# fhausmann/deepgrp

Hardware: AMD Instinct MI355X
Metric: Mbp/sec predicted (whole node) at window=200 stride=50, 5-class (higher is better)
Workload: dtype f16

## Files before the change

### deepgrp_amd/csrc/gru_shared.h

```cpp
#pragma once
#include "dgrp_model.h"

typedef _Float16 half8 __attribute__((ext_vector_type(8)));
typedef float f32x16 __attribute__((ext_vector_type(16)));
typedef float f32x4 __attribute__((ext_vector_type(4)));
typedef _Float16 half4 __attribute__((ext_vector_type(4)));

#define DGRP_WG_WINDOWS 16

struct gru_rec {
    int64_t idx_off, n, out_row, nwin;
    dgrp_placement place;
    int64_t win_first;
    int64_t pad_;
};

struct gru_params {
    const uint8_t *idx;
    int64_t n, s, w0, nw;
    dgrp_placement place;
    const uint4 *pack;
    const float *ffb;
    float *out;
    void *avg;
    int avg_f32;
    int T, C, nfrag, mode;
    int Tp;
    int ospan;
    const struct gru_rec *recs;
    const int64_t *wg_first;
    int64_t nrec;
    int64_t avgw;
    const uint4 *pack_lo;
    int lo_tile_off;
    float zfold;
    const uint4 *pack16;
    const float *xtab;
    int xtab_off;
    const uint4 *stream;
    const uint4 *packw;
    const float *xtabw;
    int avg_up;
};

__device__ __forceinline__ float sigmoid_from_scaled(float a) { return __builtin_amdgcn_rcpf(1.0f + __builtin_amdgcn_exp2f(a)); }
__device__ __forceinline__ float tanh_from_scaled(float a) { return 1.0f - 2.0f * __builtin_amdgcn_rcpf(1.0f + __builtin_amdgcn_exp2f(a)); }
typedef float f32x2 __attribute__((ext_vector_type(2)));
__device__ __forceinline__ f32x2 rcp1p_exp2_pair(float a0, float a1)
{
    f32x2 e = { __builtin_amdgcn_exp2f(a0), __builtin_amdgcn_exp2f(a1) };
    e = e + 1.0f;
    return f32x2{ __builtin_amdgcn_rcpf(e.x), __builtin_amdgcn_rcpf(e.y) };
}
__device__ __forceinline__ float fast_tanh(float x) { return tanh_from_scaled(2.8853900817779268f * x); }

template <int N>
__device__ __forceinline__ float row_ror(float x)
{
    return __builtin_bit_cast(float, __builtin_amdgcn_update_dpp(0, __builtin_bit_cast(int, x), 0x120 | N, 0xf, 0xf, false));
}
template <int N>
__device__ __forceinline__ float row_max_ror(float x)
{
    float r;
    asm("s_nop 1\n\tv_max_f32_dpp %0, %1, %1 row_ror:%2 row_mask:0xf bank_mask:0xf" : "=v"(r) : "v"(x), "n"(N));
    return r;
}
template <int CTRL>
__device__ __forceinline__ float quad_perm(float x)
{
    return __builtin_bit_cast(float, __builtin_amdgcn_update_dpp(0, __builtin_bit_cast(int, x), CTRL, 0xf, 0xf, false));
}
__device__ __forceinline__ float row_allmax(float x)
{
    return row_max_ror<1>(row_max_ror<2>(row_max_ror<4>(row_max_ror<8>(x))));
}
__device__ __forceinline__ float row_allsum(float x)
{
    x += row_ror<8>(x); x += row_ror<4>(x); x += row_ror<2>(x); return x + row_ror<1>(x);
}

typedef __attribute__((address_space(3))) unsigned lds_u32;
typedef __attribute__((address_space(1))) unsigned glb_u32;
__device__ __forceinline__ void lds_atomic_max(unsigned *p, unsigned v)
{
    (void)__hip_atomic_fetch_max((lds_u32 *)p, v, __ATOMIC_RELAXED, __HIP_MEMORY_SCOPE_WORKGROUP);
}
__device__ __forceinline__ void global_atomic_max(unsigned *p, unsigned v)
{
    (void)__hip_atomic_fetch_max((glb_u32 *)p, v, __ATOMIC_RELAXED, __HIP_MEMORY_SCOPE_AGENT);
}

__host__ __device__ static inline int gru_lds_hbuf(int UP, int pad = 8) { return 2 * 32 * (UP + pad) * 2; }
__host__ __device__ static inline int gru_lds_dpart(int NW) { return 2 * NW * 64 * 16; }
__host__ __device__ static inline int gru_lds_seq(int Tp) { return DGRP_WG_WINDOWS * Tp; }
__host__ __device__ static inline int gru_lds_meta() { return DGRP_WG_WINDOWS * 8 + DGRP_WG_WINDOWS * 4; }

struct wg_ctx {
    _Float16 *hbuf;
    float *dpart;
    uint8_t *seqs;
    int64_t *row0s;
    int *rowoff;
    unsigned *obuf;
    int64_t wg_w, lo;
    int nvalid;
};

template <int MODE>
__device__ __forceinline__ int64_t wg_record_at(const gru_params &pin, gru_params &p, int64_t g)
{
    if (MODE == 1 || !pin.recs) return g;
    int64_t lo_r = 0, hi_r = pin.nrec;
    while (hi_r - lo_r > 1) {
        const int64_t mid = (lo_r + hi_r) >> 1;
        if (pin.wg_first[mid] <= g) lo_r = mid; else hi_r = mid;
    }
    const gru_rec rc = pin.recs[lo_r];
    p.idx = pin.idx + rc.idx_off;
    p.n = rc.n;
    if (MODE == 0) p.out = pin.out + rc.out_row * pin.C;
    p.place = rc.place;
    p.w0 = 0;
    p.nw = rc.nwin;
    p.avgw = rc.win_first;
    return g - pin.wg_first[lo_r];
}
template <int MODE>
__device__ __forceinline__ int64_t wg_record(const gru_params &pin, gru_params &p) { return wg_record_at<MODE>(pin, p, blockIdx.x); }

template <int NW, int MODE, int HPAD = 8>
__device__ __forceinline__ wg_ctx wg_setup(const gru_params &p, unsigned char *smem, int64_t bid)
{
    constexpr int UP = 32 * NW, HS = UP + HPAD;
    wg_ctx c;
    c.hbuf = reinterpret_cast<_Float16 *>(smem);
    c.dpart = reinterpret_cast<float *>(smem + gru_lds_hbuf(UP, HPAD));
    c.seqs = smem + gru_lds_hbuf(UP, HPAD) + gru_lds_dpart(NW);
    c.row0s = reinterpret_cast<int64_t *>(c.seqs + gru_lds_seq(p.Tp));
    c.rowoff = reinterpret_cast<int *>(c.row0s + DGRP_WG_WINDOWS);
    c.obuf = reinterpret_cast<unsigned *>(c.rowoff + DGRP_WG_WINDOWS);
    const int tid = threadIdx.x, T = p.T, C = p.C;
    c.wg_w = p.w0 + bid * DGRP_WG_WINDOWS;
    c.nvalid = (int)min((int64_t)DGRP_WG_WINDOWS, p.w0 + p.nw - c.wg_w);
    for (int i = tid; i < DGRP_WG_WINDOWS * T; i += 64 * NW) {
        const int wi = i / T, t = i - wi * T;
        c.seqs[wi * p.Tp + t] = wi < c.nvalid ? p.idx[(c.wg_w + wi) * p.s + t] : (uint8_t)4;
    }
    for (int i = tid; i < 32 * HS; i += 64 * NW) c.hbuf[i] = (_Float16)0.0f;
    c.lo = 0;
    if (MODE == 0) {
        const int64_t a = dgrp_place_row(p.place, c.wg_w, p.s), b = dgrp_place_row(p.place, c.wg_w + c.nvalid - 1, p.s);
        c.lo = a < b ? a : b;
        for (int i = tid; i < p.ospan * C; i += 64 * NW) c.obuf[i] = 0u;
    }
    if (tid < DGRP_WG_WINDOWS) {
        int64_t r0 = -1;
        int off = -1;
        if (tid < c.nvalid) {
            r0 = MODE == 0 ? dgrp_place_row(p.place, c.wg_w + tid, p.s) : (c.wg_w + tid - p.w0 + p.avgw) * (int64_t)T;
            if (MODE == 0 && r0 >= c.lo && r0 - c.lo + T <= p.ospan) off = (int)(r0 - c.lo);
        }
        c.row0s[tid] = r0;
        c.rowoff[tid] = off;
    }
    __syncthreads();
    return c;
}

template <int MODE>
__device__ __forceinline__ void emit_value(const gru_params &p, const wg_ctx &c, int off, int64_t row0, int t, int cls, float val)
{
    if (MODE == 0) {
        if (off >= 0) {
            lds_atomic_max(c.obuf + (off + t) * p.C + cls, __float_as_uint(val));
        } else {
            const int64_t row = row0 + t;
            if (row < p.n) global_atomic_max(reinterpret_cast<unsigned *>(p.out) + row * p.C + cls, __float_as_uint(val));
        }
    } else {
        p.out[(row0 + t) * p.C + cls] = val;
    }
}

template <int NW, int MODE>
__device__ __forceinline__ void finish_register(const gru_params &p, const wg_ctx &c, int t, int reg, float fbias, int off, int64_t row0)
{
    const int lane = threadIdx.x & 63, cls = lane & 15;
    const float *dp = c.dpart + ((size_t)(t & 1) * 4 + reg) * NW * 64 + lane;
    float sum = dp[0];
#pragma unroll
    for (int w = 1; w < NW; ++w) sum += dp[w * 64];
    const int wi = 4 * (lane >> 4) + reg;
    const float lg = cls < p.C ? sum + fbias : -INFINITY;
    float val = lg;
    if (MODE != 2) {
        const float m = row_allmax(lg);
        const float e = __builtin_amdgcn_exp2f(1.4426950408889634f * (lg - m));
        val = e * __builtin_amdgcn_rcpf(row_allsum(e));
    }
    if (cls < p.C && wi < c.nvalid) emit_value<MODE>(p, c, off, row0, t, cls, val);
}

template <int NW>
__device__ __forceinline__ void flush_image(const gru_params &p, const wg_ctx &c)
{
    __syncthreads();
    unsigned *gout = reinterpret_cast<unsigned *>(p.out) + c.lo * p.C;
    const int64_t lim = (p.n - c.lo) * p.C;
    for (int i = threadIdx.x; i < p.ospan * p.C; i += 64 * NW) {
        const unsigned v = c.obuf[i];
        if (v != 0u && i < lim) global_atomic_max(gout + i, v);
    }
}

__device__ __forceinline__ void split_avg_store_lane(const gru_params &p, int64_t wg_w, int tt, int UP, int wave, int lane, half8 a0, half8 a1,
                                                     half8 l0, half8 l1)
{
    const int64_t at = ((wg_w + (lane & 15) - p.w0 + p.avgw) * (int64_t)p.T + tt) * UP + 32 * wave + 8 * (lane >> 4);
    if (p.avg_f32) {
        float *dst = reinterpret_cast<float *>(p.avg) + at;
        typedef unsigned u32x4_ __attribute__((ext_vector_type(4)));
        const _Float16 hf = (_Float16)0.5f;
        const u32x4_ A0 = __builtin_bit_cast(u32x4_, a0), A1 = __builtin_bit_cast(u32x4_, a1);
        const u32x4_ L0 = __builtin_bit_cast(u32x4_, l0 * hf), L1 = __builtin_bit_cast(u32x4_, l1 * hf);
        float v[8];
#pragma unroll
        for (int k = 0; k < 4; ++k) {
            float f0, f1, r0, r1;
            asm("v_fma_mix_f32 %0, %1, 0.5, %2 op_sel_hi:[1,0,1]" : "=v"(f0) : "v"(A0[k]), "v"(L0[k]));
            asm("v_fma_mix_f32 %0, %1, 0.5, %2 op_sel:[1,0,1] op_sel_hi:[1,0,1]" : "=v"(f1) : "v"(A0[k]), "v"(L0[k]));
            asm("v_fma_mix_f32 %0, %1, 0.5, %2 op_sel_hi:[1,0,1]" : "=v"(r0) : "v"(A1[k]), "v"(L1[k]));
            asm("v_fma_mix_f32 %0, %1, 0.5, %2 op_sel:[1,0,1] op_sel_hi:[1,0,1]" : "=v"(r1) : "v"(A1[k]), "v"(L1[k]));
            v[2 * k] = f0 + r0;
            v[2 * k + 1] = f1 + r1;
        }
        *reinterpret_cast<f32x4 *>(dst) = f32x4{ v[0], v[1], v[2], v[3] };
        *reinterpret_cast<f32x4 *>(dst + 4) = f32x4{ v[4], v[5], v[6], v[7] };
        return;
    }
    const _Float16 hf = (_Float16)0.5f;
    const half8 av = (a0 * hf + a1 * hf) + (l0 + l1) * hf;
    *reinterpret_cast<half8 *>(reinterpret_cast<_Float16 *>(p.avg) + at) = av;
}
__device__ __forceinline__ void split_avg_store(const gru_params &p, int64_t wg_w, int tt, int UP, int wave, half8 a0, half8 a1,
                                                half8 l0, half8 l1)
{
    split_avg_store_lane(p, wg_w, tt, UP, wave, threadIdx.x & 63, a0, a1, l0, l1);
}

struct split_gate_tmp { float er, e2, g, A, zt, d, n; };
template <bool ONERCP, int OP>
__device__ __forceinline__ void split_gate_op(split_gate_tmp &t, float ar, float ag, float az, float ax, float &s)
{
#pragma clang fp contract(off)
    if constexpr (OP == 0) t.er = __builtin_amdgcn_exp2f(ar);
    else if constexpr (OP == 1) t.e2 = __builtin_amdgcn_exp2f(az);
    else if constexpr (OP == 2) t.er = t.er + 1.0f;
    else if constexpr (OP == 3) t.er = __builtin_amdgcn_rcpf(t.er);
    else if constexpr (OP == 4) t.g = __builtin_fmaf(t.er, ag, ax);
    else if constexpr (OP == 5) t.A = __builtin_amdgcn_exp2f(t.g);
    else if constexpr (OP == 6) t.A = t.A + 1.0f;
    else if constexpr (ONERCP) {
        if constexpr (OP == 7) t.zt = __builtin_fmaf(0.5f, t.e2, 1.0f);
        else if constexpr (OP == 8) t.d = t.A * t.zt;
        else if constexpr (OP == 9) t.n = __builtin_fmaf(s, t.A, -t.e2);
        else if constexpr (OP == 10) t.d = __builtin_amdgcn_rcpf(t.d);
        else s = t.n * t.d;
    } else {
        if constexpr (OP == 7) t.zt = t.e2 + 1.0f;
        else if constexpr (OP == 8) t.d = __builtin_amdgcn_rcpf(t.A);
        else if constexpr (OP == 9) t.n = __builtin_fmaf(-2.0f, t.d, 1.0f);
        else if constexpr (OP == 10) t.zt = __builtin_amdgcn_rcpf(t.zt);
        else { const float df = s - t.n; s = __builtin_fmaf(t.zt, df, t.n); }
    }
}
#define DGRP_SPLIT_GATE_OPS 12
template <bool ONERCP>
__device__ __forceinline__ float split_gate_chain(float ar, float ag, float az, float ax, float s)
{
    split_gate_tmp t;
    split_gate_op<ONERCP, 0>(t, ar, ag, az, ax, s); split_gate_op<ONERCP, 1>(t, ar, ag, az, ax, s);
    split_gate_op<ONERCP, 2>(t, ar, ag, az, ax, s); split_gate_op<ONERCP, 3>(t, ar, ag, az, ax, s);
    split_gate_op<ONERCP, 4>(t, ar, ag, az, ax, s); split_gate_op<ONERCP, 5>(t, ar, ag, az, ax, s);
    split_gate_op<ONERCP, 6>(t, ar, ag, az, ax, s); split_gate_op<ONERCP, 7>(t, ar, ag, az, ax, s);
    split_gate_op<ONERCP, 8>(t, ar, ag, az, ax, s); split_gate_op<ONERCP, 9>(t, ar, ag, az, ax, s);
    split_gate_op<ONERCP, 10>(t, ar, ag, az, ax, s); split_gate_op<ONERCP, 11>(t, ar, ag, az, ax, s);
    return s;
}
template <bool ONERCP> __device__ __forceinline__ float split_state_h(float s)
{
#pragma clang fp contract(off)
    return ONERCP ? s + 1.0f : s;
}
__device__ __forceinline__ uint2 split_pack4(const float h[4])
{
    uint2 r;
    asm("v_cvt_pk_f16_f32 %0, %1, %2" : "=v"(r.x) : "v"(h[0]), "v"(h[1]));
    asm("v_cvt_pk_f16_f32 %0, %1, %2" : "=v"(r.y) : "v"(h[2]), "v"(h[3]));
    return r;
}
__device__ __forceinline__ void split_residual4(float h[4], uint2 hi)
{
    asm("v_fma_mix_f32 %0, %1, -1.0, %0 op_sel_hi:[1,0,0]" : "+v"(h[0]) : "v"(hi.x));
    asm("v_fma_mix_f32 %0, %1, -1.0, %0 op_sel:[1,0,0] op_sel_hi:[1,0,0]" : "+v"(h[1]) : "v"(hi.x));
    asm("v_fma_mix_f32 %0, %1, -1.0, %0 op_sel_hi:[1,0,0]" : "+v"(h[2]) : "v"(hi.y));
    asm("v_fma_mix_f32 %0, %1, -1.0, %0 op_sel:[1,0,0] op_sel_hi:[1,0,0]" : "+v"(h[3]) : "v"(hi.y));
}
__device__ __forceinline__ void split_hi_lo4(const float h[4], uint2 &hv, uint2 &lv)
{
    float r[4] = { h[0], h[1], h[2], h[3] };
    hv = split_pack4(r);
    split_residual4(r, hv);
    lv = split_pack4(r);
}

__device__ __forceinline__ float wave_half_sum(float h, float half)
{
#pragma clang fp contract(off)
    float t = half * h;
    asm("s_nop 1\n\tv_fmac_f32_dpp %0, %1, %2 row_ror:8 row_mask:0xf bank_mask:0xf" : "+v"(t) : "v"(h), "v"(half));
    return t;
}

__device__ __forceinline__ void split_lstm_cell(float ai, float af, float ac, float ao, float &c, float &h)
{
#pragma clang fp contract(off)
    const float ig = __builtin_amdgcn_rcpf(1.0f + __builtin_amdgcn_exp2f(ai));
    const float fg = __builtin_amdgcn_rcpf(1.0f + __builtin_amdgcn_exp2f(af));
    const float tc = __builtin_fmaf(-2.0f, __builtin_amdgcn_rcpf(1.0f + __builtin_amdgcn_exp2f(ac)), 1.0f);
    const float it = ig * tc;
    c = __builtin_fmaf(fg, c, it);
    const float og = __builtin_amdgcn_rcpf(1.0f + __builtin_amdgcn_exp2f(ao));
    const float e2 = __builtin_amdgcn_exp2f(2.8853900817779268f * c);
    const float th = __builtin_fmaf(-2.0f, __builtin_amdgcn_rcpf(1.0f + e2), 1.0f);
    h = og * th;
}
```

### deepgrp_amd/csrc/gru_split2.hip

```cpp
#include "gru_shared.h"
#include <mutex>
#include <type_traits>

typedef unsigned u32x4 __attribute__((ext_vector_type(4)));

namespace {

constexpr int NW = 4, UP = 128, KS = 4, HPAD = 16, HS = UP + HPAD;
constexpr int XT_PITCH = 4 * 128 * 4 + 32;

struct split2_weights {
    u32x4 hi[3][KS][2], lo[3][KS][2];
    u32x4 Bd_hi, Bd_lo;
};

#define LOAD2(a, pa, b, pb)                                                                                             \
    asm volatile("global_load_dwordx4 %0, %2, off\n\tglobal_load_dwordx4 %1, %3, off\n\ts_waitcnt vmcnt(0)"            \
                 : "=&a"(a), "=&a"(b) : "v"(pa), "v"(pb) : "memory")

#define MFMA_R(acc, Wf, b) asm volatile("v_mfma_f32_16x16x32_f16 %0, %1, %2, %0" : "+v"(acc) : "a"(Wf), "v"(b))
#define MFMA_D(acc, a, Wf) asm volatile("v_mfma_f32_16x16x32_f16 %0, %1, %2, %0" : "+v"(acc) : "v"(a), "a"(Wf))
#define MFMA_DZ(acc, a, Wf) asm volatile("v_mfma_f32_16x16x32_f16 %0, %1, %2, 0" : "=&v"(acc) : "v"(a), "a"(Wf))

struct tile_state {
    gru_params p;
    wg_ctx ctx;
    unsigned hcur, hnxt, lcur, lnxt;
    unsigned myseq;
    float h[16];
    f32x4 ar[4], ag[4], az[4], ax[4];
    f32x4 dpl;
    unsigned tabf, tabr;
    half8 f0h[2], f0l[2];
    int p_off;
    int64_t p_row0;
    bool pr_on;
};

template <int MODE, bool ONERCP>
__global__ void __launch_bounds__(256) __attribute__((amdgpu_waves_per_eu(1, 1))) gru_split2_kernel(const gru_params pin, int half_bytes)
{
    extern __shared__ __attribute__((aligned(16))) unsigned char smem[];
    const int tid = threadIdx.x;
    const int lane = tid & 63;
    const int wave = __builtin_amdgcn_readfirstlane(tid >> 6);
    const int T = pin.T, C = pin.C;

    split2_weights W;
    {
        const uint4 *p16 = pin.pack16 + (size_t)wave * 48 * 64 + lane;
#pragma unroll
        for (int g = 0; g < 3; ++g)
#pragma unroll
            for (int ks = 0; ks < KS; ++ks) {
                LOAD2(W.hi[g][ks][0], p16 + (size_t)(g * 8 + ks * 2) * 64, W.hi[g][ks][1], p16 + (size_t)(g * 8 + ks * 2 + 1) * 64);
                LOAD2(W.lo[g][ks][0], p16 + (size_t)(24 + g * 8 + ks * 2) * 64, W.lo[g][ks][1], p16 + (size_t)(24 + g * 8 + ks * 2 + 1) * 64);
            }
        const uint4 *mypack = pin.pack + (size_t)wave * pin.nfrag * 64 + lane;
        LOAD2(W.Bd_hi, mypack + (size_t)(3 * (2 * KS + 1) + 1) * 64, W.Bd_lo, mypack + (size_t)(3 * (2 * KS + 1) + 2) * 64);
    }
    for (int i = tid; i < 5 * 512; i += 256)
        *reinterpret_cast<float *>(smem + pin.xtab_off + (i / 512) * XT_PITCH + (i % 512) * 4) = pin.xtab[i];

    const int wi = lane & 15, q4 = lane >> 4;
    const int cls = lane & 15;
    const float fbias = cls < C ? pin.ffb[cls] : 0.0f;
    const int pwi = 4 * (lane >> 4) + wave;
    const unsigned frag_lane = (unsigned)(wi * HS + 8 * q4) * 2;
    const unsigned dense_lane = (unsigned)(wi * HS + 32 * wave + 8 * q4) * 2;
    const unsigned pub_lane = (unsigned)(wi * HS + 32 * wave + 4 * q4) * 2;
    const unsigned tab_lane = (unsigned)pin.xtab_off + (unsigned)(32 * wave + 4 * q4) * 4;

    tile_state S0, S1;
    auto setup = [&](tile_state &Z, int x) {
        unsigned char *base = smem + (size_t)x * half_bytes;
        _Float16 *lbuf = reinterpret_cast<_Float16 *>(base + pin.lo_tile_off);
        for (int i = tid; i < 32 * HS; i += 256) lbuf[i] = (_Float16)0.0f;
        Z.p = pin;
        const int64_t bid = wg_record_at<MODE>(pin, Z.p, 2 * (int64_t)blockIdx.x + x);
        Z.ctx = wg_setup<NW, MODE, HPAD>(Z.p, base, bid);
        Z.hcur = (unsigned)x * half_bytes;
        Z.hnxt = Z.hcur + 32 * HS * 2;
        Z.lcur = (unsigned)x * half_bytes + pin.lo_tile_off;
        Z.lnxt = Z.lcur + 32 * HS * 2;
        Z.myseq = (unsigned)(Z.ctx.seqs - smem) + wi * pin.Tp;
#pragma unroll
        for (int i = 0; i < 16; ++i) Z.h[i] = ONERCP ? -1.0f : 0.0f;
        Z.p_off = Z.ctx.rowoff[pwi];
        Z.p_row0 = Z.ctx.row0s[pwi];
        Z.pr_on = cls < C && pwi < Z.ctx.nvalid;
    };
    setup(S0, 0);
    setup(S1, 1);

    auto lds16 = [&](unsigned off) -> half8 { return *reinterpret_cast<const half8 *>(smem + off); };
    auto ldsf4 = [&](unsigned off) -> f32x4 { return *reinterpret_cast<const f32x4 *>(smem + off); };
    auto tab_rows = [&](tile_state &Z, uint32_t bf, uint32_t br) {
        bf = bf < 4 ? bf : 4;
        br = br < 4 ? 3 - br : 4;
        Z.tabf = tab_lane + bf * XT_PITCH;
        Z.tabr = tab_lane + br * XT_PITCH;
    };
    auto acc_init = [&](tile_state &Z, int g, int sub) {
        const f32x4 v = ldsf4(((sub & 1) ? Z.tabr : Z.tabf) + g * 512 + (sub >> 1) * 64);
        if (g == 0) Z.ar[sub] = v; else if (g == 1) Z.ag[sub] = v; else Z.az[sub] = v;
    };

    struct frag_ring { half8 h[2][2], l[2][2]; };
    struct dense_ops { half8 a0, a1, l0, l1; };
    struct fin_state { float d[NW], lg, m, e, s; };
    auto phase = [&](auto do_x, auto do_y, auto do_f, tile_state &X, tile_state &Y, int tx, int ty) __attribute__((always_inline)) {
        constexpr bool DO_X = decltype(do_x)::value, DO_Y = decltype(do_y)::value, DO_F = decltype(do_f)::value;
        frag_ring F;
        dense_ops D;
        fin_state fs;
        split_gate_tmp gt[16];
        float pbh[4][4];
        uint2 pbhv[4], pblv[4];
        uint32_t xp_bf = 4, xp_br = 4;
        const int td = ty - 1;
        const int tf = tx - 2;
        if constexpr (DO_X) { F.h[0][0] = X.f0h[0]; F.h[0][1] = X.f0h[1]; F.l[0][0] = X.f0l[0]; F.l[0][1] = X.f0l[1]; }
#define GAP __builtin_amdgcn_sched_barrier(0);
#define M_K(ks, n)                                                                                               \
    if constexpr (DO_X) {                                                                                        \
        constexpr int ps_ = (n) / 12, g_ = ((n) % 12) / 4, uh_ = ((n) % 4) / 2, rh_ = (n) % 2, sub_ = 2 * uh_ + rh_; \
        const half8 &b_ = ps_ == 1 ? F.l[(ks) & 1][rh_] : F.h[(ks) & 1][rh_];                                    \
        const u32x4 &w_ = ps_ == 2 ? W.lo[g_][ks][uh_] : W.hi[g_][ks][uh_];                                      \
        if constexpr (g_ == 0) MFMA_R(X.ar[sub_], w_, b_);                                                       \
        else if constexpr (g_ == 1) MFMA_R(X.ag[sub_], w_, b_);                                                  \
        else MFMA_R(X.az[sub_], w_, b_);                                                                         \
    }
#define M_D(i)                                                                                                   \
    if constexpr (DO_X) {                                                                                        \
        if constexpr ((i) == 0) MFMA_DZ(X.dpl, D.a0, W.Bd_hi);                                                   \
        else if constexpr ((i) == 1) MFMA_D(X.dpl, D.a1, W.Bd_hi);                                               \
        else if constexpr ((i) == 2) MFMA_D(X.dpl, D.a0, W.Bd_lo);                                               \
        else if constexpr ((i) == 3) MFMA_D(X.dpl, D.a1, W.Bd_lo);                                               \
        else if constexpr ((i) == 4) MFMA_D(X.dpl, D.l0, W.Bd_hi);                                               \
        else MFMA_D(X.dpl, D.l1, W.Bd_hi);                                                                       \
    }
#define PF(ks)                                                                                                   \
    if constexpr (DO_X) {                                                                                        \
        F.h[(ks) & 1][0] = lds16(X.hcur + frag_lane + 64 * (ks)); F.h[(ks) & 1][1] = lds16(X.hcur + frag_lane + 16 * HS * 2 + 64 * (ks)); \
        F.l[(ks) & 1][0] = lds16(X.lcur + frag_lane + 64 * (ks)); F.l[(ks) & 1][1] = lds16(X.lcur + frag_lane + 16 * HS * 2 + 64 * (ks)); \
    }
#define RDD                                                                                                      \
    if constexpr (DO_X) {                                                                                        \
        D.a0 = lds16(X.hcur + dense_lane); D.a1 = lds16(X.hcur + dense_lane + 16 * HS * 2);                      \
        D.l0 = lds16(X.lcur + dense_lane); D.l1 = lds16(X.lcur + dense_lane + 16 * HS * 2);                      \
        if (MODE == 2 && tx > 0 && (lane & 15) < X.ctx.nvalid)                                                   \
            split_avg_store(X.p, X.ctx.wg_w, tx - 1, UP, wave, D.a0, D.a1, D.l0, D.l1);                          \
    }
#define AXL(sub) \
    if constexpr (DO_Y) Y.ax[sub] = ldsf4((((sub) & 1) ? Y.tabr : Y.tabf) + 3 * 512 + ((sub) >> 1) * 64);
#define DS(i)                                                                                                    \
    if constexpr (DO_Y) Y.ctx.dpart[((size_t)(td & 1) * 4 * NW + wave) * 64 + lane + (i) * NW * 64] = Y.dpl[i];
#define G(e, op) \
    if constexpr (DO_Y) split_gate_op<ONERCP, op>(gt[e], Y.ar[(e) / 4][(e) % 4], Y.ag[(e) / 4][(e) % 4], Y.az[(e) / 4][(e) % 4], Y.ax[(e) / 4][(e) % 4], Y.h[e]);
#define PB(g, op)                                                                                                \
    if constexpr (DO_Y) {                                                                                        \
        if constexpr ((op) == 0) {                                                                               \
            pbh[g][0] = split_state_h<ONERCP>(Y.h[4 * (g)]); pbh[g][1] = split_state_h<ONERCP>(Y.h[4 * (g) + 1]); \
            pbh[g][2] = split_state_h<ONERCP>(Y.h[4 * (g) + 2]); pbh[g][3] = split_state_h<ONERCP>(Y.h[4 * (g) + 3]); \
        } else if constexpr ((op) == 1) {                                                                        \
            pbhv[g] = split_pack4(pbh[g]);                                                                       \
        } else if constexpr ((op) == 2) {                                                                        \
            split_residual4(pbh[g], pbhv[g]);                                                                    \
        } else if constexpr ((op) == 3) {                                                                        \
            pblv[g] = split_pack4(pbh[g]);                                                                       \
        } else {                                                                                                 \
            *reinterpret_cast<uint2 *>(smem + Y.hnxt + pub_lane + ((g) & 1) * 16 * HS * 2 + ((g) >> 1) * 32) = pbhv[g]; \
            *reinterpret_cast<uint2 *>(smem + Y.lnxt + pub_lane + ((g) & 1) * 16 * HS * 2 + ((g) >> 1) * 32) = pblv[g]; \
        }                                                                                                        \
    }
#define BAR                                                                                                      \
    if constexpr (DO_Y) {                                                                                        \
        asm volatile("s_waitcnt lgkmcnt(0)\n\ts_barrier" ::: "memory");                                          \
        unsigned sw_ = Y.hcur; Y.hcur = Y.hnxt; Y.hnxt = sw_;                                                    \
        sw_ = Y.lcur; Y.lcur = Y.lnxt; Y.lnxt = sw_;                                                             \
    }
#define RD0                                                                                                      \
    if constexpr (DO_Y) {                                                                                        \
        Y.f0h[0] = lds16(Y.hcur + frag_lane); Y.f0h[1] = lds16(Y.hcur + frag_lane + 16 * HS * 2);                \
        Y.f0l[0] = lds16(Y.lcur + frag_lane); Y.f0l[1] = lds16(Y.lcur + frag_lane + 16 * HS * 2);                \
    }
#define XP(op)                                                                                                   \
    if constexpr (DO_Y) {                                                                                        \
        if constexpr ((op) == 0) { xp_bf = smem[Y.myseq + ty + 1]; xp_br = smem[Y.myseq + T - 2 - ty]; }                       \
        else tab_rows(Y, xp_bf, xp_br);                                                                          \
    }
#define CI(g, sub) \
    if constexpr (DO_Y) acc_init(Y, g, sub);
#define FN(op)                                                                                                   \
    if constexpr (DO_F) {                                                                                        \
        if constexpr ((op) == 0) {                                                                               \
            const float *dp_ = X.ctx.dpart + ((size_t)(tf & 1) * 4 + wave) * NW * 64 + lane;                     \
            fs.d[0] = dp_[0]; fs.d[1] = dp_[64]; fs.d[2] = dp_[128]; fs.d[3] = dp_[192];                         \
        } else if constexpr ((op) == 1) {                                                                        \
            const float sum_ = ((fs.d[0] + fs.d[1]) + fs.d[2]) + fs.d[3];                                        \
            fs.lg = cls < C ? sum_ + fbias : -INFINITY;                                                          \
        } else if constexpr ((op) == 2) { if (MODE != 2) fs.m = row_max_ror<8>(fs.lg); }                         \
        else if constexpr ((op) == 3) { if (MODE != 2) fs.m = row_max_ror<4>(fs.m); }                            \
        else if constexpr ((op) == 4) { if (MODE != 2) fs.m = row_max_ror<2>(fs.m); }                            \
        else if constexpr ((op) == 5) { if (MODE != 2) fs.m = row_max_ror<1>(fs.m); }                            \
        else if constexpr ((op) == 6) { if (MODE != 2) fs.e = __builtin_amdgcn_exp2f(1.4426950408889634f * (fs.lg - fs.m)); } \
        else if constexpr ((op) == 7) { if (MODE != 2) fs.s = fs.e + row_ror<8>(fs.e); }                         \
        else if constexpr ((op) == 8) { if (MODE != 2) fs.s += row_ror<4>(fs.s); }                               \
        else if constexpr ((op) == 9) { if (MODE != 2) fs.s += row_ror<2>(fs.s); }                               \
        else if constexpr ((op) == 10) { if (MODE != 2) fs.s += row_ror<1>(fs.s); }                              \
        else if constexpr ((op) == 11) { if (MODE != 2) fs.e *= __builtin_amdgcn_rcpf(fs.s); }                   \
        else { if (X.pr_on && tf >= 0) emit_value<MODE>(X.p, X.ctx, X.p_off, X.p_row0, tf, cls, MODE == 2 ? fs.lg : fs.e); } \
    }
#include "gru_split2_phase.inc"
#undef GAP
#undef M_K
#undef M_D
#undef PF
#undef RDD
#undef AXL
#undef DS
#undef G
#undef PB
#undef BAR
#undef RD0
#undef XP
#undef CI
#undef FN
    };
    const std::true_type yes;
    const std::false_type no;

    auto first_step = [&](tile_state &Z) {
        tab_rows(Z, smem[Z.myseq], smem[Z.myseq + T - 1]);
#pragma unroll
        for (int g = 0; g < 3; ++g)
#pragma unroll
            for (int sub = 0; sub < 4; ++sub) acc_init(Z, g, sub);
        Z.f0h[0] = lds16(Z.hcur + frag_lane); Z.f0h[1] = lds16(Z.hcur + frag_lane + 16 * HS * 2);
        Z.f0l[0] = lds16(Z.lcur + frag_lane); Z.f0l[1] = lds16(Z.lcur + frag_lane + 16 * HS * 2);
    };
    first_step(S0);
    first_step(S1);
    phase(yes, no, no, S0, S1, 0, 0);
#define EDGE_PAD do { asm volatile("s_nop 15\n\ts_nop 7"); __builtin_amdgcn_sched_barrier(0); } while (0)
    EDGE_PAD;
    for (int t = 0; t + 1 < T; ++t) {
        phase(yes, yes, yes, S1, S0, t, t);
        phase(yes, yes, yes, S0, S1, t + 1, t);
        EDGE_PAD;
    }
    phase(yes, yes, yes, S1, S0, T - 1, T - 1);
    phase(no, yes, yes, S0, S1, T, T - 1);

    auto drain = [&](tile_state &Z, bool prev_open) {
        const half8 a0 = lds16(Z.hcur + dense_lane), a1 = lds16(Z.hcur + dense_lane + 16 * HS * 2);
        const half8 l0 = lds16(Z.lcur + dense_lane), l1 = lds16(Z.lcur + dense_lane + 16 * HS * 2);
        if (MODE == 2 && (lane & 15) < Z.ctx.nvalid) split_avg_store(Z.p, Z.ctx.wg_w, T - 1, UP, wave, a0, a1, l0, l1);
        f32x4 d;
        MFMA_DZ(d, a0, W.Bd_hi); MFMA_D(d, a1, W.Bd_hi); MFMA_D(d, a0, W.Bd_lo); MFMA_D(d, a1, W.Bd_lo); MFMA_D(d, l0, W.Bd_hi); MFMA_D(d, l1, W.Bd_hi);
        asm volatile("s_nop 15\n\ts_nop 7" : "+v"(d));
        float *dw = Z.ctx.dpart + ((size_t)((T - 1) & 1) * 4 * NW + wave) * 64 + lane;
#pragma unroll
        for (int reg = 0; reg < 4; ++reg) dw[reg * NW * 64] = d[reg];
        __syncthreads();
        if (prev_open && T > 1) finish_register<NW, MODE>(Z.p, Z.ctx, T - 2, wave, fbias, Z.p_off, Z.p_row0);
        finish_register<NW, MODE>(Z.p, Z.ctx, T - 1, wave, fbias, Z.p_off, Z.p_row0);
        if (MODE == 0 && pin.ospan > 0) flush_image<NW>(Z.p, Z.ctx);
    };
    drain(S0, false);
    drain(S1, true);
}

template <int MODE, bool ONERCP>
int launch_split2(const gru_params &p, int64_t groups, int half_bytes, hipStream_t stream)
{
    static std::once_flag configured;
    static hipError_t cfg_err = hipSuccess;
    std::call_once(configured, [] { cfg_err = hipFuncSetAttribute((const void *)gru_split2_kernel<MODE, ONERCP>, hipFuncAttributeMaxDynamicSharedMemorySize, 160 * 1024); });
    DGRP_HIP(cfg_err);
    hipLaunchKernelGGL((gru_split2_kernel<MODE, ONERCP>), dim3((unsigned)((groups + 1) / 2)), dim3(256), (size_t)2 * half_bytes + 5 * XT_PITCH, stream, p, half_bytes);
    DGRP_LAUNCH_CHECK();
    return DGRP_OK;
}

}

int dgrp_split2_launch(const gru_params &p, int64_t groups, int half_bytes, bool onercp, hipStream_t stream)
{
    if (onercp)
        return p.mode == 0 ? launch_split2<0, true>(p, groups, half_bytes, stream)
             : p.mode == 1 ? launch_split2<1, true>(p, groups, half_bytes, stream) : launch_split2<2, true>(p, groups, half_bytes, stream);
    return p.mode == 0 ? launch_split2<0, false>(p, groups, half_bytes, stream)
         : p.mode == 1 ? launch_split2<1, false>(p, groups, half_bytes, stream) : launch_split2<2, false>(p, groups, half_bytes, stream);
}
```

Before: 554.5.

## Make split2 GRU kernel persistent over tile pairs with one block per CU

Measured after the change: 560.1 (median of 6 runs). +1.0%, better.

```diff
diff --git a/deepgrp_amd/csrc/gru_shared.h b/deepgrp_amd/csrc/gru_shared.h
--- a/deepgrp_amd/csrc/gru_shared.h
+++ b/deepgrp_amd/csrc/gru_shared.h
@@ -184,9 +184,10 @@
 }
 
 template <int NW, int MODE>
-__device__ __forceinline__ void finish_register(const gru_params &p, const wg_ctx &c, int t, int reg, float fbias, int off, int64_t row0)
-{
-    const int lane = threadIdx.x & 63, cls = lane & 15;
+__device__ __forceinline__ void finish_register(const gru_params &p, const wg_ctx &c, int t, int reg, float fbias, int off, int64_t row0,
+                                                int lane = threadIdx.x & 63)
+{
+    const int cls = lane & 15;
     const float *dp = c.dpart + ((size_t)(t & 1) * 4 + reg) * NW * 64 + lane;
     float sum = dp[0];
 #pragma unroll
@@ -203,12 +204,12 @@
 }
 
 template <int NW>
-__device__ __forceinline__ void flush_image(const gru_params &p, const wg_ctx &c)
+__device__ __forceinline__ void flush_image(const gru_params &p, const wg_ctx &c, int tid = threadIdx.x)
 {
     __syncthreads();
     unsigned *gout = reinterpret_cast<unsigned *>(p.out) + c.lo * p.C;
     const int64_t lim = (p.n - c.lo) * p.C;
-    for (int i = threadIdx.x; i < p.ospan * p.C; i += 64 * NW) {
+    for (int i = tid; i < p.ospan * p.C; i += 64 * NW) {
         const unsigned v = c.obuf[i];
         if (v != 0u && i < lim) global_atomic_max(gout + i, v);
     }
diff --git a/deepgrp_amd/csrc/gru_split2.hip b/deepgrp_amd/csrc/gru_split2.hip
--- a/deepgrp_amd/csrc/gru_split2.hip
+++ b/deepgrp_amd/csrc/gru_split2.hip
@@ -1,4 +1,5 @@
 #include "gru_shared.h"
+#include <cstddef>
 #include <mutex>
 #include <type_traits>
 
@@ -15,8 +16,9 @@
 };
 
 #define LOAD2(a, pa, b, pb)                                                                                             \
-    asm volatile("global_load_dwordx4 %0, %2, off\n\tglobal_load_dwordx4 %1, %3, off\n\ts_waitcnt vmcnt(0)"            \
+    asm volatile("global_load_dwordx4 %0, %2, off\n\tglobal_load_dwordx4 %1, %3, off"                                   \
                  : "=&a"(a), "=&a"(b) : "v"(pa), "v"(pb) : "memory")
+#define LOAD_WAIT asm volatile("s_waitcnt vmcnt(0)" ::: "memory")
 
 #define MFMA_R(acc, Wf, b) asm volatile("v_mfma_f32_16x16x32_f16 %0, %1, %2, %0" : "+v"(acc) : "a"(Wf), "v"(b))
 #define MFMA_D(acc, a, Wf) asm volatile("v_mfma_f32_16x16x32_f16 %0, %1, %2, %0" : "+v"(acc) : "v"(a), "a"(Wf))
@@ -37,9 +39,92 @@
     bool pr_on;
 };
 
+__device__ __forceinline__ int64_t split2_uniform(int64_t v)
+{
+    const unsigned lo = (unsigned)__builtin_amdgcn_readfirstlane((int)(uint64_t)v), hi = (unsigned)__builtin_amdgcn_readfirstlane((int)((uint64_t)v >> 32));
+    return (int64_t)(((uint64_t)hi << 32) | lo);
+}
+
+template <int MODE>
+__device__ __forceinline__ wg_ctx split2_tile_setup(const gru_params &p, unsigned char *base, int64_t bid, int tid, unsigned &seq_row0, unsigned &seq_pitch)
+{
+    wg_ctx c;
+    c.hbuf = reinterpret_cast<_Float16 *>(base);
+    c.dpart = reinterpret_cast<float *>(base + gru_lds_hbuf(UP, HPAD));
+    c.seqs = base + gru_lds_hbuf(UP, HPAD) + gru_lds_dpart(NW);
+    c.row0s = reinterpret_cast<int64_t *>(c.seqs + gru_lds_seq(p.Tp));
+    c.rowoff = reinterpret_cast<int *>(c.row0s + DGRP_WG_WINDOWS);
+    c.obuf = reinterpret_cast<unsigned *>(c.rowoff + DGRP_WG_WINDOWS);
+    const int T = p.T, C = p.C;
+    c.wg_w = split2_uniform(p.w0 + bid * DGRP_WG_WINDOWS);
+    c.nvalid = __builtin_amdgcn_readfirstlane((int)min((int64_t)DGRP_WG_WINDOWS, p.w0 + p.nw - c.wg_w));
+    if ((DGRP_WG_WINDOWS - 1) * p.s + T + 15 <= (int64_t)DGRP_WG_WINDOWS * p.Tp) {
+        const uint8_t *src = p.idx + c.wg_w * p.s;
+        const int have = c.nvalid > 0 ? (c.nvalid - 1) * (int)p.s + T : 0;
+        const int sh = (int)(reinterpret_cast<uintptr_t>(src) & 15);
+        const int head = min(have, (16 - sh) & 15);
+        const int nbody = (have - head) >> 4, tail0 = head + 16 * nbody;
+#pragma nounroll
+        for (int i = tid; i < nbody; i += 64 * NW)
+            *reinterpret_cast<uint4 *>(c.seqs + sh + head + 16 * i) = *reinterpret_cast<const uint4 *>(src + head + 16 * i);
+#pragma nounroll
+        for (int i = tid; i < head + have - tail0; i += 64 * NW) {
+            const int j = i < head ? i : tail0 + (i - head);
+            c.seqs[sh + j] = src[j];
+        }
+        seq_row0 = (unsigned)sh;
+        seq_pitch = (unsigned)p.s;
+    } else {
+#pragma nounroll
+        for (int i = tid; i < DGRP_WG_WINDOWS * T; i += 64 * NW) {
+            const int wi = i / T, t = i - wi * T;
+            c.seqs[wi * p.Tp + t] = wi < c.nvalid ? p.idx[(c.wg_w + wi) * p.s + t] : (uint8_t)4;
+        }
+        seq_row0 = 0;
+        seq_pitch = (unsigned)p.Tp;
+    }
+    unsigned z0 = 0u;
+    asm volatile("" : "+v"(z0));
+    const uint4 zero = { z0, z0, z0, z0 };
+#pragma nounroll
+    for (int i = tid; i < 32 * HS * 2 / 16; i += 64 * NW) {
+        reinterpret_cast<uint4 *>(base)[i] = zero;
+        reinterpret_cast<uint4 *>(base + p.lo_tile_off)[i] = zero;
+    }
+    c.lo = 0;
+    if (MODE == 0) {
+        const int64_t a = dgrp_place_row(p.place, c.wg_w, p.s), b = dgrp_place_row(p.place, c.wg_w + c.nvalid - 1, p.s);
+        c.lo = split2_uniform(a < b ? a : b);
+        const int words = p.ospan * C;
+#pragma nounroll
+        for (int i = tid; i < words / 4; i += 64 * NW) reinterpret_cast<uint4 *>(c.obuf)[i] = zero;
+        if (tid < (words & 3)) c.obuf[(words & ~3) + tid] = 0u;
+    }
+    if (tid < DGRP_WG_WINDOWS) {
+        int64_t r0 = -1;
+        int off = -1;
+        if (tid < c.nvalid) {
+            r0 = MODE == 0 ? dgrp_place_row(p.place, c.wg_w + tid, p.s) : (c.wg_w + tid - p.w0 + p.avgw) * (int64_t)T;
+            if (MODE == 0 && r0 >= c.lo && r0 - c.lo + T <= p.ospan) off = (int)(r0 - c.lo);
+        }
+        c.row0s[tid] = r0;
+        c.rowoff[tid] = off;
+    }
+    return c;
+}
+
+struct split2_args {
+    gru_params p;
+    int half_bytes;
+    int npairs;
+};
+
 template <int MODE, bool ONERCP>
-__global__ void __launch_bounds__(256) __attribute__((amdgpu_waves_per_eu(1, 1))) gru_split2_kernel(const gru_params pin, int half_bytes)
-{
+__global__ void __launch_bounds__(256) __attribute__((amdgpu_waves_per_eu(1, 1))) gru_split2_kernel(const split2_args args)
+{
+    static_assert(offsetof(split2_args, p) == 0 && sizeof(gru_params) % 4 == 0 && offsetof(split2_args, half_bytes) % 4 == 0 &&
+                  offsetof(split2_args, npairs) % 4 == 0, "the pair loop reads the argument as 32-bit words");
+    const gru_params &pin = args.p;
     extern __shared__ __attribute__((aligned(16))) unsigned char smem[];
     const int tid = threadIdx.x;
     const int lane = tid & 63;
@@ -58,6 +143,7 @@
             }
         const uint4 *mypack = pin.pack + (size_t)wave * pin.nfrag * 64 + lane;
         LOAD2(W.Bd_hi, mypack + (size_t)(3 * (2 * KS + 1) + 1) * 64, W.Bd_lo, mypack + (size_t)(3 * (2 * KS + 1) + 2) * 64);
+        LOAD_WAIT;
     }
     for (int i = tid; i < 5 * 512; i += 256)
         *reinterpret_cast<float *>(smem + pin.xtab_off + (i / 512) * XT_PITCH + (i % 512) * 4) = pin.xtab[i];
@@ -65,33 +151,32 @@
     const int wi = lane & 15, q4 = lane >> 4;
     const int cls = lane & 15;
     const float fbias = cls < C ? pin.ffb[cls] : 0.0f;
-    const int pwi = 4 * (lane >> 4) + wave;
     const unsigned frag_lane = (unsigned)(wi * HS + 8 * q4) * 2;
     const unsigned dense_lane = (unsigned)(wi * HS + 32 * wave + 8 * q4) * 2;
     const unsigned pub_lane = (unsigned)(wi * HS + 32 * wave + 4 * q4) * 2;
     const unsigned tab_lane = (unsigned)pin.xtab_off + (unsigned)(32 * wave + 4 * q4) * 4;
 
     tile_state S0, S1;
-    auto setup = [&](tile_state &Z, int x) {
-        unsigned char *base = smem + (size_t)x * half_bytes;
-        _Float16 *lbuf = reinterpret_cast<_Float16 *>(base + pin.lo_tile_off);
-        for (int i = tid; i < 32 * HS; i += 256) lbuf[i] = (_Float16)0.0f;
-        Z.p = pin;
-        const int64_t bid = wg_record_at<MODE>(pin, Z.p, 2 * (int64_t)blockIdx.x + x);
-        Z.ctx = wg_setup<NW, MODE, HPAD>(Z.p, base, bid);
-        Z.hcur = (unsigned)x * half_bytes;
+    auto setup = [&](tile_state &Z, const gru_params &pk, int tid_k, int half_k, int pair, int x) {
+        unsigned char *base = smem + (size_t)x * half_k;
+        Z.p = pk;
+        const int64_t bid = wg_record_at<MODE>(pk, Z.p, 2 * (int64_t)pair + x);
+        unsigned seq_row0, seq_pitch;
+        Z.ctx = split2_tile_setup<MODE>(Z.p, base, bid, tid_k, seq_row0, seq_pitch);
+        Z.hcur = (unsigned)x * half_k;
         Z.hnxt = Z.hcur + 32 * HS * 2;
-        Z.lcur = (unsigned)x * half_bytes + pin.lo_tile_off;
+        Z.lcur = (unsigned)x * half_k + pk.lo_tile_off;
         Z.lnxt = Z.lcur + 32 * HS * 2;
-        Z.myseq = (unsigned)(Z.ctx.seqs - smem) + wi * pin.Tp;
+        Z.myseq = (unsigned)(Z.ctx.seqs - smem) + seq_row0 + (tid_k & 15) * seq_pitch;
 #pragma unroll
         for (int i = 0; i < 16; ++i) Z.h[i] = ONERCP ? -1.0f : 0.0f;
-        Z.p_off = Z.ctx.rowoff[pwi];
-        Z.p_row0 = Z.ctx.row0s[pwi];
-        Z.pr_on = cls < C && pwi < Z.ctx.nvalid;
-    };
-    setup(S0, 0);
-    setup(S1, 1);
+    };
+    auto placement = [&](tile_state &Z, int tid_k) {
+        const int pwi_k = 4 * ((tid_k & 63) >> 4) + wave;
+        Z.p_off = Z.ctx.rowoff[pwi_k];
+        Z.p_row0 = Z.ctx.row0s[pwi_k];
+        Z.pr_on = cls < C && pwi_k < Z.ctx.nvalid;
+    };
 
     auto lds16 = [&](unsigned off) -> half8 { return *reinterpret_cast<const half8 *>(smem + off); };
     auto ldsf4 = [&](unsigned off) -> f32x4 { return *reinterpret_cast<const f32x4 *>(smem + off); };
@@ -240,6 +325,21 @@
         Z.f0h[0] = lds16(Z.hcur + frag_lane); Z.f0h[1] = lds16(Z.hcur + frag_lane + 16 * HS * 2);
         Z.f0l[0] = lds16(Z.lcur + frag_lane); Z.f0l[1] = lds16(Z.lcur + frag_lane + 16 * HS * 2);
     };
+    for (int pair = blockIdx.x;;) {
+    const __attribute__((address_space(4))) unsigned *kargs = (const __attribute__((address_space(4))) unsigned *)__builtin_amdgcn_kernarg_segment_ptr();
+    asm volatile("" : "+s"(kargs));
+    struct { unsigned w[sizeof(gru_params) / 4]; } kraw;
+#pragma unroll
+    for (unsigned i = 0; i < sizeof(gru_params) / 4; ++i) kraw.w[i] = kargs[offsetof(split2_args, p) / 4 + i];
+    const gru_params pk = __builtin_bit_cast(gru_params, kraw);
+    const int half_k = (int)kargs[offsetof(split2_args, half_bytes) / 4];
+    int tid_k = 64 * wave + lane;
+    asm volatile("" : "+v"(tid_k));
+    setup(S0, pk, tid_k, half_k, pair, 0);
+    setup(S1, pk, tid_k, half_k, pair, 1);
+    __syncthreads();
+    placement(S0, tid_k);
+    placement(S1, tid_k);
     first_step(S0);
     first_step(S1);
     phase(yes, no, no, S0, S1, 0, 0);
@@ -253,23 +353,49 @@
     phase(yes, yes, yes, S1, S0, T - 1, T - 1);
     phase(no, yes, yes, S0, S1, T, T - 1);
 
-    auto drain = [&](tile_state &Z, bool prev_open) {
+    auto drain = [&](tile_state &Z, bool prev_open, int tid_d) {
+        const int lane_d = tid_d & 63;
         const half8 a0 = lds16(Z.hcur + dense_lane), a1 = lds16(Z.hcur + dense_lane + 16 * HS * 2);
         const half8 l0 = lds16(Z.lcur + dense_lane), l1 = lds16(Z.lcur + dense_lane + 16 * HS * 2);
-        if (MODE == 2 && (lane & 15) < Z.ctx.nvalid) split_avg_store(Z.p, Z.ctx.wg_w, T - 1, UP, wave, a0, a1, l0, l1);
+        if (MODE == 2 && (lane_d & 15) < Z.ctx.nvalid) split_avg_store_lane(Z.p, Z.ctx.wg_w, T - 1, UP, wave, lane_d, a0, a1, l0, l1);
         f32x4 d;
         MFMA_DZ(d, a0, W.Bd_hi); MFMA_D(d, a1, W.Bd_hi); MFMA_D(d, a0, W.Bd_lo); MFMA_D(d, a1, W.Bd_lo); MFMA_D(d, l0, W.Bd_hi); MFMA_D(d, l1, W.Bd_hi);
         asm volatile("s_nop 15\n\ts_nop 7" : "+v"(d));
-        float *dw = Z.ctx.dpart + ((size_t)((T - 1) & 1) * 4 * NW + wave) * 64 + lane;
+        float *dw = Z.ctx.dpart + ((size_t)((T - 1) & 1) * 4 * NW + wave) * 64 + lane_d;
 #pragma unroll
         for (int reg = 0; reg < 4; ++reg) dw[reg * NW * 64] = d[reg];
         __syncthreads();
-        if (prev_open && T > 1) finish_register<NW, MODE>(Z.p, Z.ctx, T - 2, wave, fbias, Z.p_off, Z.p_row0);
-        finish_register<NW, MODE>(Z.p, Z.ctx, T - 1, wave, fbias, Z.p_off, Z.p_row0);
-        if (MODE == 0 && pin.ospan > 0) flush_image<NW>(Z.p, Z.ctx);
-    };
-    drain(S0, false);
-    drain(S1, true);
+        if (prev_open && T > 1) finish_register<NW, MODE>(Z.p, Z.ctx, T - 2, wave, fbias, Z.p_off, Z.p_row0, lane_d);
+        finish_register<NW, MODE>(Z.p, Z.ctx, T - 1, wave, fbias, Z.p_off, Z.p_row0, lane_d);
+        if (MODE == 0 && Z.p.ospan > 0) flush_image<NW>(Z.p, Z.ctx, tid_d);
+    };
+    int tid_d = 64 * wave + lane;
+    asm volatile("" : "+v"(tid_d));
+    drain(S0, false, tid_d);
+    drain(S1, true, tid_d);
+    __syncthreads();
+    EDGE_PAD;
+    pair += (int)gridDim.x;
+    if (pair >= (int)kargs[offsetof(split2_args, npairs) / 4]) break;
+    }
+}
+
+static int split2_cu_count(int *cus)
+{
+    static std::mutex mu;
+    static int known[64];
+    int dev = 0;
+    DGRP_HIP(hipGetDevice(&dev));
+    std::lock_guard<std::mutex> lock(mu);
+    if (dev < 0 || dev >= 64 || known[dev] == 0) {
+        int n = 0;
+        DGRP_HIP(hipDeviceGetAttribute(&n, hipDeviceAttributeMultiprocessorCount, dev));
+        if (n < 1) n = 1;
+        if (dev < 0 || dev >= 64) { *cus = n; return DGRP_OK; }
+        known[dev] = n;
+    }
+    *cus = known[dev];
+    return DGRP_OK;
 }
 
 template <int MODE, bool ONERCP>
@@ -279,7 +405,12 @@
     static hipError_t cfg_err = hipSuccess;
     std::call_once(configured, [] { cfg_err = hipFuncSetAttribute((const void *)gru_split2_kernel<MODE, ONERCP>, hipFuncAttributeMaxDynamicSharedMemorySize, 160 * 1024); });
     DGRP_HIP(cfg_err);
-    hipLaunchKernelGGL((gru_split2_kernel<MODE, ONERCP>), dim3((unsigned)((groups + 1) / 2)), dim3(256), (size_t)2 * half_bytes + 5 * XT_PITCH, stream, p, half_bytes);
+    const int64_t npairs = (groups + 1) / 2;
+    int cus = 0;
+    if (const int rc = split2_cu_count(&cus)) return rc;
+    const int64_t grid = npairs < cus ? npairs : cus;
+    DGRP_REQUIRE(npairs >= 1 && npairs <= 0x7fff0000, "gru_split2_kernel: tile pairs out of range");
+    hipLaunchKernelGGL((gru_split2_kernel<MODE, ONERCP>), dim3((unsigned)grid), dim3(256), (size_t)2 * half_bytes + 5 * XT_PITCH, stream, split2_args{ p, half_bytes, (int)npairs });
     DGRP_LAUNCH_CHECK();
     return DGRP_OK;
 }
```
